# linum-uqam/ViT-OCM-WMSegmentation

Hardware: AMD Instinct MI355X
Metric: OCM tiles/s (224x224, ViT-S/16 attention-map inference) (higher is better)
Workload: dtype bf16x3

## Files before the change

vit-ocm-wmsegmentation_amd/csrc/engine.hip:

```cpp
#include <stdarg.h>
#include <stdio.h>
#include <string.h>

#include <atomic>
#include <mutex>
#include <string>
#include <vector>

#include "host_common.h"
#include "launch.h"
#include "dev_knobs.h"
#include "attn_plan.h"

static thread_local std::string g_err;

int ocm_fail(int code, const char *fmt, ...) {
    char buf[512];
    va_list ap;
    va_start(ap, fmt);
    vsnprintf(buf, sizeof buf, fmt, ap);
    va_end(ap);
    g_err = buf;
    return code;
}
// ... 330 lines not shown
    w.bytes = off;
    return w;
}

extern "C" size_t ocm_vit_workspace_bytes(const ocm_vit_t *h, int32_t batch, int32_t n_tokens) {
    if (!h || batch <= 0 || n_tokens <= 1) return 0;
    return carve(h, batch, n_tokens, nullptr).bytes;
}

static int check_ws(const ocm_vit *h, int batch, int n, void *ws, size_t ws_bytes) {
    if (!ws) return fail(OCM_ENOMEM, "workspace is null");
    if ((uintptr_t)ws & 255) return fail(OCM_EINVAL, "workspace must be 256-byte aligned");
    const size_t need = carve(h, batch, n, nullptr).bytes;
    if (ws_bytes < need) return fail(OCM_ENOMEM, "workspace too small: %zu < %zu bytes", ws_bytes, need);
    return OCM_OK;
}

static int run_attention(const ocm_vit *h, const Workspace &w, int batch, int n, bool attn_only, float *out_attn, float *out_qkv,
                         const int32_t *query_rows, int n_rows, float *out_rows, const char *qkv_w, const float *qkv_b,
                         const LnFold &ln, hipStream_t s) {
    const int H = h->H, np = ocm_n_pad_for(h->prec, n), pc = h->prec;
    const float scale = h->cfg.qk_scale;
    const bool want_v = !(attn_only && !out_qkv);
    if (!h->mfma_heads()) {
        float *qkv = out_qkv ? out_qkv : w.qkv32;
        { PROF(OCM_K_QKV, s); HIP_TRY(launch_qkv(pc, w.xn, qkv_w, qkv_b, nullptr, nullptr, nullptr, qkv, batch, n, np, H, h->hd, want_v, s, ln)); }
        { PROF(OCM_K_ATTN, s); HIP_TRY(launch_attention_generic(pc, qkv, attn_only ? nullptr : w.ctx, out_attn, query_rows, n_rows, out_rows, batch, n, H, h->hd, scale, s)); }
        return OCM_OK;
    }
    void *vt_dst = want_v ? w.vt : nullptr;
    { PROF(OCM_K_QKV, s); HIP_TRY(launch_qkv(pc, w.xn, qkv_w, qkv_b, w.q, w.k, vt_dst, out_qkv, batch, n, np, H, h->hd, want_v, s, ln)); }
    if (out_rows && !out_attn) { PROF(OCM_K_PROBS, s); HIP_TRY(launch_attention_rows(pc, w.q, w.k, query_rows, n_rows, out_rows, batch, n, np, H, scale, s, h->hd)); }
    if (attn_only && !out_attn) return OCM_OK;
    { PROF(OCM_K_ATTN, s); HIP_TRY(launch_attention(pc, w.q, w.k, w.vt, attn_only ? nullptr : w.ctx, out_attn ? w.lse : nullptr, batch, n, np, H, scale, s, h->hd, w.kpart, w.kpart_bytes)); }
    if (out_attn) {
        PROF(OCM_K_PROBS, s);
        HIP_TRY(launch_attention_probs(pc, w.q, w.k, w.lse, out_attn, batch, n, np, H, scale, s, h->hd, query_rows, n_rows, out_rows));
    }
    return OCM_OK;
}

static int run_block(const ocm_vit *h, int i, const Workspace &w, float *x, int batch, int n, bool attn_only,
                     float *out_attn, float *out_qkv, const int32_t *query_rows, int n_rows, float *out_rows,
                     hipStream_t s, bool xn_ready = false, const float *next_g = nullptr, const float *next_b = nullptr,
                     bool *xn_out = nullptr) {
    const BlockP &bp = h->blk[i];
    const int D = h->D, T = batch * n;
    const float eps = h->cfg.ln_eps;
    const int pc = h->prec, lnk = ln_kind_of_prec(pc);
    const long t128 = (long)((T + 127) / 128) * (D / 128);
    const int fuse_opt = h->opt[OCM_OPT_FUSE_LN];
    const bool fuse_ln = linear_resid_ln_supported(D) && fuse_opt != 1 && ((T >= 8192 && t128 < 512) || fuse_opt == 2);
    if (xn_out) *xn_out = false;
    if (!xn_ready) { PROF(OCM_K_LN, s); HIP_TRY(launch_layernorm(x, h->ptr<float>(bp.ln1_g), h->ptr<float>(bp.ln1_b), w.xn, lnk, T, D, eps, s)); }
    if (int rc = run_attention(h, w, batch, n, attn_only, out_attn, out_qkv, query_rows, n_rows, out_rows, h->ptr<char>(bp.qkv_w),
                               h->ptr<float>(bp.qkv_b), LnFold(), s))
        return rc;
    if (attn_only) return OCM_OK;
    if (fuse_ln) {
        PROF(OCM_K_PROJ, s);
        HIP_TRY(launch_linear_resid_ln(pc, w.ctx, h->ptr<char>(bp.proj_w), h->ptr<float>(bp.proj_b), x, x, h->ptr<float>(bp.ln2_g), h->ptr<float>(bp.ln2_b), w.xn, T, D, D, eps, s));
    } else {
        { PROF(OCM_K_PROJ, s); HIP_TRY(launch_linear(pc, w.ctx, h->ptr<char>(bp.proj_w), h->ptr<float>(bp.proj_b), x, x, T, D, D, OCM_EPI_BIAS_RESID_F32, s)); }
        { PROF(OCM_K_LN, s); HIP_TRY(launch_layernorm(x, h->ptr<float>(bp.ln2_g), h->ptr<float>(bp.ln2_b), w.xn, lnk, T, D, eps, s)); }
    }
    { PROF(OCM_K_FC1, s); HIP_TRY(launch_linear(pc, w.xn, h->ptr<char>(bp.fc1_w), h->ptr<float>(bp.fc1_b), nullptr, w.hid, T, h->M, D, OCM_EPI_BIAS_GELU_BF16, s)); }
    if (fuse_ln && next_g && next_b) {
        PROF(OCM_K_FC2, s);
        HIP_TRY(launch_linear_resid_ln(pc, w.hid, h->ptr<char>(bp.fc2_w), h->ptr<float>(bp.fc2_b), x, x, next_g, next_b, w.xn, T, D, h->M, eps, s));
        if (xn_out) *xn_out = true;
// ... 640 lines not shown
```

vit-ocm-wmsegmentation_amd/csrc/gemm_kernels.h:

```cpp
#pragma once
#include <type_traits>
#include "gemm_core.h"
#include "launch.h"
#include "gemm_plan.h"
#include "dev_knobs.h"

int ocm_wt_mask();

template <GemmTile T>
using CfgOf = GemmCfg<GEMM_TILES[T].bm, GEMM_TILES[T].bn, GEMM_TILES[T].waves_m, GEMM_TILES[T].waves_n, GEMM_TILES[T].mf16>;
typedef CfgOf<T128x128> Cfg128x128;
typedef CfgOf<T128x128q> Cfg128x128q;
typedef CfgOf<T128x128q16> Cfg128x128q16;
typedef CfgOf<T128x128m16> Cfg128x128m16;
typedef CfgOf<T160x128q16> Cfg160x128q16;
typedef CfgOf<T256x256m16> Cfg256x256m16;
typedef CfgOf<T64x128> Cfg64x128;
typedef CfgOf<T64x128w> Cfg64x128w;
typedef CfgOf<T64x64> Cfg64x64;
typedef CfgOf<T256x256> Cfg256x256;
typedef CfgOf<T256x128> Cfg256x128;
typedef CfgOf<T128x192> Cfg128x192;
typedef CfgOf<T128x96> Cfg128x96;

// ... 958 lines not shown
};

struct EpiPatch {
    static constexpr bool ROWTAB = false;
    const float *bias, *pos;
    float *x;
    int M, P, ntok, D;
    const float *mask, *mask_tok;
    StatsOut so;
    template <class Cfg>
    __device__ __forceinline__ void run(const float *C, int m0, int n0, const f32x2 *, const f32x2 *) const {
        constexpr int BM = Cfg::BM, BN = Cfg::BN, NT = Cfg::NT, CPR = BN / 4;
        if (so.stats) return run_stats<Cfg>(C, m0, n0);
#pragma unroll 4
        for (int q = threadIdx.x; q < BM * CPR; q += NT) {
            const int row = q / CPR, col = (q - row * CPR) * 4;
            const int m = m0 + row, n = n0 + col;
            if (m >= M || n >= D) continue;
            const int b = m / P, t = m - b * P;
            f32x4 v = *(const f32x4 *)(C + row * BN + col);
            if (mask) {
                const float w = mask[m], omw = 1.0f - w;
                const f32x4 tk = *(const f32x4 *)(mask_tok + n);
#pragma unroll
                for (int e = 0; e < 4; ++e) v[e] = v[e] * omw + tk[e] * w;
            }
            v += *(const f32x4 *)(pos + (int64_t)(1 + t) * D + n);
            *(f32x4 *)(x + ((int64_t)b * ntok + 1 + t) * D + n) = v;
        }
    }
    template <class Cfg>
    __device__ __forceinline__ void run_stats(const float *C, int m0, int n0) const {
        constexpr int BM = Cfg::BM, BN = Cfg::BN, NT = Cfg::NT, CPR = BN / 4;
        static_assert((BM * CPR) % NT == 0 && CPR <= 32 && (CPR & (CPR - 1)) == 0, "CPR lanes of one wave half own a row");
        const int sl = threadIdx.x & (CPR - 1), col = sl * 4, n = n0 + col;
        const bool nok = n < D;
        const int nc = min(n, D - 4);
#pragma unroll 1
        for (int row = threadIdx.x / CPR; row < BM; row += NT / CPR) {
            const int m = m0 + row;
            const bool ok = nok && m < M;
            const int mc = min(m, M - 1);
            const int b = mc / P, t = mc - b * P;
            f32x4 v = *(const f32x4 *)(C + row * BN + col);
            if (mask) {
                const float w = mask[mc], omw = 1.0f - w;
                const f32x4 tk = *(const f32x4 *)(mask_tok + nc);
#pragma unroll
                for (int e = 0; e < 4; ++e) v[e] = v[e] * omw + tk[e] * w;
            }
            v += *(const f32x4 *)(pos + (int64_t)(1 + t) * D + nc);
            const int64_t xrow = (int64_t)b * ntok + 1 + t;
            const float sh = so.tok_shift ? so.tok_shift[1 + t] : 0.f;
            float s1 = 0.f, s2 = 0.f;
            if (ok) {
                *(f32x4 *)(x + xrow * D + n) = v;
                if (so.shift && n0 == 0 && sl == 0) so.shift[xrow] = sh;
                v -= sh;
                bf16x4 hi, lo;
                split4(v, hi, lo);
                char *g = (char *)so.xs + xrow * D * 4 + sp_off(n);
                *(bf16x4 *)g = hi;
                *(bf16x4 *)(g + 64) = lo;
                s1 = (v[0] + v[1]) + (v[2] + v[3]);
                s2 = fmaf(v[0], v[0], fmaf(v[1], v[1], fmaf(v[2], v[2], v[3] * v[3])));
            }
#pragma unroll
            for (int o = CPR / 2; o > 0; o >>= 1) {
                s1 += __shfl_xor(s1, o, 64);
                s2 += __shfl_xor(s2, o, 64);
            }
            if (m < M && sl < BN / 64 && n0 + 64 * sl < D) {
                const f32x2 val = {sl ? 0.f : s1, sl ? 0.f : s2};
                *((f32x2 *)so.stats + xrow * (D >> 6) + (n0 >> 6) + sl) = val;
            }
        }
    }
};

template <class E>
hipError_t launch_patch_e(const PatchArgs &pa, const E *w, const float *bias, const float *pos, float *x, int dim,
                                 hipStream_t s, const StatsOut &so) {
    const int P = pa.hp * pa.wp, M = pa.batch * P, K = pa.chans * pa.p * pa.p;
    PatchLoader<E> al{pa.image, pa.sb, pa.sc, pa.sy, pa.origins, P, pa.wp, pa.p, pa.p * pa.p};
    EpiPatch epi{bias, pos, x, M, P, P + 1, dim, pa.mask, pa.mask_tok, so};
    if (K % Elem<E>::KROW) return hipErrorInvalidValue;
    const int ks = gemm_ct_steps<KsLinearReg>(K / Elem<E>::KROW);
    if constexpr (Elem<E>::MODE == 2)
        if (dim % 128 == 0 && M > 64 && M <= 1024) return launch_gemm<Cfg64x128w, E, false>(al, w, K, M, dim, K, epi, s, ks);
    if (dim % 128 == 0 && M > 64) return launch_gemm<Cfg64x128, E, false>(al, w, K, M, dim, K, epi, s, ks);
    return launch_gemm<Cfg64x64, E, false>(al, w, K, M, dim, K, epi, s, ks);
}
```

vit-ocm-wmsegmentation_amd/csrc/kernels_attn.hip:

```cpp
#include <stdlib.h>

#include "launch.h"

#define LOG2E 1.4426950408889634f
int ocm_wt_mask();
#include "dev_knobs.h"
#include "attn_plan.h"
#define OCM_VMCNT_ATTN(n) asm volatile("s_waitcnt vmcnt(%0)" ::"n"(n) : "memory")

#ifndef OCM_DEFER_MAX
#define OCM_DEFER_MAX 8.0f
#endif
__device__ __forceinline__ float defer_max_update(float &m, float cand) {
    if (__any(cand > m + OCM_DEFER_MAX)) {
        const float mn = fmaxf(m, cand);
        const float alpha = fast_exp2(m - mn);
        m = mn;
        return alpha;
    }
    return 1.0f;
}

template <bool WANT_O, int HD = 64>
__global__ __launch_bounds__(256, HD == 64 ? 3 : 2) void attn_fwd_kernel(const bf16 *__restrict__ Q, const bf16 *__restrict__ Kk,
// ... 531 lines not shown
#pragma unroll
            for (int c = 0; c < 4; ++c) {
                const f32x4 kf = *(const f32x4 *)(Kb + (int64_t)key * HD + 32 * hf + 16 * h + 4 * c);
#pragma unroll
                for (int e = 0; e < 4; ++e) S = mfma32f(qf[hf][c][e], kf[e], S);
            }
        if (kt * 32 + r < N) {
#pragma unroll
            for (int e = 0; e < 16; ++e) {
                const int qrow = q0 + acc_row32(e, h);
                if (qrow < N) out[(int64_t)qrow * N + kt * 32 + r] = fast_exp2(S[e] * scale2 - lr[e]);
            }
        }
    }
}

#ifdef OCM_GEMM_STAMPS
__device__ unsigned long long g_astamps[1024 * 8 * 16];
extern "C" int ocm_debug_stamps_attn(unsigned long long *host, int n) {
    return (int)hipMemcpyFromSymbol(host, HIP_SYMBOL(g_astamps), (size_t)n * 8);
}
#define ASTAMP(k)                                                                                                    \
    do {                                                                                                             \
        const unsigned wg_ = blockIdx.y * gridDim.x + blockIdx.x;                                                    \
        if ((threadIdx.x & 63) == 0 && wg_ < 1024 && (k) < 16)                                                       \
            g_astamps[(wg_ * 8 + (threadIdx.x >> 6 & 7)) * 16 + (k)] = __builtin_readcyclecounter();                 \
    } while (0)
#define ASTAMP_RT(k)                                                                                                 \
    do {                                                                                                             \
        const unsigned wg_ = blockIdx.y * gridDim.x + blockIdx.x;                                                    \
        if ((threadIdx.x & 63) == 0 && wg_ < 1024)                                                                   \
            g_astamps[(wg_ * 8 + (threadIdx.x >> 6 & 7)) * 16 + (k)] = wall_clock64();                               \
    } while (0)
#else
#define ASTAMP(k) ((void)0)
#define ASTAMP_RT(k) ((void)0)
#endif


template <int NQ>
__device__ __forceinline__ void x3_load_q(const char *qp, int h, bf16x8 (&qh)[NQ], bf16x8 (&ql)[NQ]) {
#pragma unroll
    for (int s = 0; s < NQ; ++s) {
        const char *p = qp + (s >> 1) * 128 + ((s & 1) * 16 + 8 * h) * 2;
        qh[s] = *(const bf16x8 *)p;
        ql[s] = *(const bf16x8 *)(p + 64);
    }
}

template <int HD, int NW, int KP, int VP>
__device__ __forceinline__ void x3_piece_offsets(int lane, int wave, int npad, int (&voffK)[KP], int (&voffV)[VP ? VP : 1]) {
    const int lrow = lane >> 3, slot = lane & 7;
#pragma unroll
    for (int j = 0; j < KP; ++j) {
        const int pc = j * NW + wave, rho = (pc & 3) * 8 + lrow;
        voffK[j] = rho * (HD * 4) + (pc >> 2) * 128 + ((slot ^ ((rho >> 1) & 7)) << 4);
    }
#pragma unroll
    for (int j = 0; j < VP; ++j) {
        const int rho = (j * NW + wave) * 8 + lrow;
        voffV[j] = rho * npad * 4 + ((slot ^ ((rho >> 1) & 7)) << 4);
    }
}
#if defined(__HIP_DEVICE_COMPILE__)
typedef __attribute__((address_space(3))) void *lds_ptr;
template <int HD>
__device__ __forceinline__ auto x3_tile_rsrc(const char *base, int npad) {
    return __builtin_amdgcn_make_buffer_rsrc((void *)base, 0, (unsigned)(npad * HD * 4), 0x00020000);
}
// ... 197 lines not shown
    }
    if (qrow < N) {
        if (lse2 && h == 0) lse2[(int64_t)bh * N + qrow] = m + __log2f(lt);
        if (WANT_O) {
            const float inv = 1.0f / lt;
            const int b = bh / H, head = bh - b * H;
            char *dst = ctx + ((int64_t)b * N + qrow) * (H * HD) * 4 + head * (HD * 4);
#pragma unroll
            for (int db = 0; db < ND; ++db)
#pragma unroll
                for (int g = 0; g < 4; ++g) {
                    f32x4 o;
#pragma unroll
                    for (int e = 0; e < 4; ++e) o[e] = O[db][4 * g + e] * inv;
                    bf16x4 oh, ol;
                    split4(o, oh, ol);
                    char *p = dst + db * 128 + (8 * g + 4 * h) * 2;
                    if (wt) {
                        const f32x2 dh = __builtin_bit_cast(f32x2, oh), dl = __builtin_bit_cast(f32x2, ol);
                        asm volatile("global_store_dwordx2 %0, %1, off sc1\n\ts_nop 1" ::"v"(p), "v"(dh) : "memory");
                        asm volatile("global_store_dwordx2 %0, %1, off sc1\n\ts_nop 1" ::"v"(p + 64), "v"(dl) : "memory");
                    } else {
                        *(bf16x4 *)p = oh;
                        *(bf16x4 *)(p + 64) = ol;
                    }
                }
        }
    }
    ASTAMP(15);
    ASTAMP_RT(13);
}


template <bool WANT_O>
__global__ __launch_bounds__(256, 3) void attn_fwd_x3_pp_kernel(const char *__restrict__ Q, const char *__restrict__ Kk,
                                                               const char *__restrict__ Vt, char *__restrict__ ctx,
                                                               float *__restrict__ lse2, int N, int npad, int H, float scale2) {
    constexpr int NW = 4, HD = 64, KB = HD * 128, KP = 8 / NW, VP = WANT_O ? 8 / NW : 0;
    __shared__ __attribute__((aligned(1024))) char smem[6 * KB];
    const int tid = threadIdx.x, lane = tid & 63;
    const int wave = __builtin_amdgcn_readfirstlane(tid >> 6);
    const int r = lane & 31, h = lane >> 5;
    int qblk, bh;
    xcd_remap2(qblk, bh);
    const int q0 = (qblk * NW + wave) * 32;
    const bool active = q0 < N;
    const char *Qb = Q + (int64_t)bh * npad * (HD * 4);
    const char *Kb = Kk + (int64_t)bh * npad * (HD * 4);
    const char *Vb = Vt + (int64_t)bh * HD * npad * 4;
    const int nt = (N + 31) >> 5;

    bf16x8 qh[4], ql[4];
    x3_load_q(Qb + (int64_t)min(q0 + r, N - 1) * (HD * 4), h, qh, ql);
    int voffK[KP], voffV[VP ? VP : 1];
    x3_piece_offsets<HD, NW, KP, VP>(lane, wave, npad, voffK, voffV);
#if defined(__HIP_DEVICE_COMPILE__)
    const auto rsK = x3_tile_rsrc<HD>(Kb, npad), rsV = x3_tile_rsrc<HD>(Vb, npad);
#define OCM_PP_DMA_K(t, slot)                                                                                        \
    do {                                                                                                             \
        _Pragma("unroll") for (int j = 0; j < KP; ++j)                                                               \
            __builtin_amdgcn_raw_ptr_buffer_load_lds(rsK, (lds_ptr)(smem + (slot) * KB + (j * NW + wave) * 1024), 16, \
                                                     voffK[j], (t) * (32 * HD * 4), 0, 0);                           \
    } while (0)
#define OCM_PP_DMA_V(t, slot)                                                                                              \
    do {                                                                                                                   \
        _Pragma("unroll") for (int j = 0; j < VP; ++j)                                                                     \
            __builtin_amdgcn_raw_ptr_buffer_load_lds(rsV, (lds_ptr)(smem + (3 + (slot)) * KB + (j * NW + wave) * 1024), 16, \
                                                     voffV[j], (t) * 128, 0, 0);                                           \
    } while (0)
#else
#define OCM_PP_DMA_K(t, slot) (void)0
#define OCM_PP_DMA_V(t, slot) (void)0
#endif
    OCM_PP_DMA_K(0, 0);
    if (nt > 1) OCM_PP_DMA_K(1, 1);
    if (WANT_O) OCM_PP_DMA_V(0, 0);
    if (nt > 2) OCM_PP_DMA_K(2, 2);
    if (WANT_O && nt > 1) OCM_PP_DMA_V(1, 1);
    __builtin_amdgcn_s_waitcnt(0x0F70);
    auto block_barrier = [&]() {
        __builtin_amdgcn_sched_barrier(0);
        asm volatile("s_waitcnt lgkmcnt(0)" ::: "memory");
        __builtin_amdgcn_s_barrier();
        asm volatile("" ::: "memory");
        __builtin_amdgcn_sched_barrier(0);
    };
    block_barrier();

    f32x16 O[2], S;
    bf16x8 ph[2], pl[2];
#pragma unroll
    for (int e = 0; e < 16; ++e) O[0][e] = O[1][e] = S[e] = 0.f;
#pragma unroll
    for (int s2 = 0; s2 < 2; ++s2)
#pragma unroll
        for (int e = 0; e < 8; ++e) ph[s2][e] = pl[s2][e] = (bf16)0.f;
    float m = -INFINITY, l = 0.f;
    const int pr = pi_row(r);
    const int first_pad = N - (nt - 1) * 32;

    auto qk = [&](int ks) {
        const char *Kt = smem + ks * KB;
#pragma unroll
        for (int e = 0; e < 16; ++e) S[e] = 0.f;
#pragma unroll
        for (int s = 0; s < 4; ++s) {
            const char *kp = Kt + (s >> 1) * 4096;
            const bf16x8 kh = *(const bf16x8 *)(kp + lds_off(pr, (s & 1) * 2 + h));
            const bf16x8 kl = *(const bf16x8 *)(kp + lds_off(pr, 4 + (s & 1) * 2 + h));
            S = mfma32x3(kh, kl, qh[s], ql[s], S);
        }
    };
    auto Mblk = [&](int vs, int ks, bool more) {
        if (WANT_O) {
            const char *Vtile = smem + (3 + vs) * KB;
#pragma unroll
            for (int s2 = 0; s2 < 2; ++s2)
#pragma unroll
                for (int db = 0; db < 2; ++db) {
                    const char *vp = Vtile + db * 32 * 128;
                    const bf16x8 vh = *(const bf16x8 *)(vp + lds_off(r, 2 * s2 + h));
                    const bf16x8 vl = *(const bf16x8 *)(vp + lds_off(r, 4 + 2 * s2 + h));
                    O[db] = mfma32x3(vh, vl, ph[s2], pl[s2], O[db]);
                }
        }
        if (more) qk(ks);
    };
    auto Vblk = [&](bool last_of_seq) {
        if (last_of_seq && first_pad < 32) x3_mask_pad_keys(S, first_pad, h);
        const float alpha = x3_softmax(S, scale2, m, l);
        if (WANT_O) {
            x3_rescale(O, alpha);
#pragma unroll
            for (int s2 = 0; s2 < 2; ++s2) x3_split_p(S, s2, ph[s2], pl[s2]);
        }
    };

    if (active) {
        qk(0);
        Vblk(nt == 1);
    }
    block_barrier();

    int s0 = 0, s1 = 1;
    for (int kt = 0; kt < nt; ++kt) {
        const int s2n = s1 == 2 ? 0 : s1 + 1;
        if (kt + 3 < nt) OCM_PP_DMA_K(kt + 3, s0);
        if (WANT_O && kt + 2 < nt) OCM_PP_DMA_V(kt + 2, s2n);
        const bool last = kt + 1 == nt;
        if (WANT_O && last && first_pad < 32) {
            x3_zero_pad_keys<HD, 64>(smem + (3 + s0) * KB, tid >> 2, tid & 3, first_pad);
            block_barrier();
        }
        if (active) {
            Mblk(s0, s1, !last);
            if (!last) Vblk(kt + 2 == nt);
        }
        if (kt + 3 < nt)
            OCM_VMCNT_ATTN(KP + VP);
        else if (WANT_O && kt + 2 < nt)
            OCM_VMCNT_ATTN(VP);
        else
            OCM_VMCNT_ATTN(0);
        block_barrier();
        s0 = s1;
        s1 = s2n;
    }
#undef OCM_PP_DMA_K
#undef OCM_PP_DMA_V

    if (!active) return;
    const float lt = l + __shfl_xor(l, 32, 64);
    const int qrow = q0 + r;
    if (lse2 && h == 0 && qrow < N) lse2[(int64_t)bh * N + qrow] = m + __log2f(lt);
    if (WANT_O) {
        const float inv = 1.0f / lt;
        const int b = bh / H, head = bh - b * H;
        char *dst = ctx + ((int64_t)b * N + min(qrow, N - 1)) * (H * HD) * 4 + head * (HD * 4);
#pragma unroll
        for (int db = 0; db < 2; ++db)
#pragma unroll
            for (int g = 0; g < 4; g += 2) {
                f32x4 oa, ob;
#pragma unroll
                for (int e = 0; e < 4; ++e) {
                    oa[e] = O[db][4 * g + e] * inv;
                    ob[e] = O[db][4 * g + 4 + e] * inv;
                }
                bf16x4 ah, al, bhh, bl;
                split4(oa, ah, al);
                split4(ob, bhh, bl);
                uint2 ahu = __builtin_bit_cast(uint2, ah), alu = __builtin_bit_cast(uint2, al);
                uint2 bhu = __builtin_bit_cast(uint2, bhh), blu = __builtin_bit_cast(uint2, bl);
                auto sw = [](unsigned &x, unsigned &y) {
                    const auto rr = __builtin_amdgcn_permlane32_swap(x, y, false, false);
                    x = rr[0];
                    y = rr[1];
                };
                sw(ahu.x, bhu.x);
                sw(ahu.y, bhu.y);
                sw(alu.x, blu.x);
                sw(alu.y, blu.y);
                if (qrow < N) {
                    char *p = dst + db * 128 + (8 * g + 8 * h) * 2;
                    *(uint4 *)p = make_uint4(ahu.x, ahu.y, bhu.x, bhu.y);
                    *(uint4 *)(p + 64) = make_uint4(alu.x, alu.y, blu.x, blu.y);
                }
            }
    }
}

template <bool WANT_O>
__global__ __launch_bounds__(256) void attn_fwd_x3_ws_kernel(const char *__restrict__ Q, const char *__restrict__ Kk,
                                                            const char *__restrict__ Vt, char *__restrict__ ctx,
                                                            float *__restrict__ lse2, int N, int npad, int H, float scale2) {
    constexpr int HD = 64, KB = HD * 128, SLOT = 2 * KB;
    extern __shared__ __attribute__((aligned(1024))) char smem[];
    const int tid = threadIdx.x, lane = tid & 63;
    const int wave = __builtin_amdgcn_readfirstlane(tid >> 6);
    const int r = lane & 31, h = lane >> 5;
    const int qt = blockIdx.x, bh = blockIdx.y;
    const int q0 = qt * 32;
    const char *Qb = Q + (int64_t)bh * npad * (HD * 4);
    const char *Kb = Kk + (int64_t)bh * npad * (HD * 4);
    const char *Vb = Vt + (int64_t)bh * HD * npad * 4;
    const int nt = (N + 31) >> 5;
    char *mine = smem + wave * 2 * SLOT;

    bf16x8 qh[4], ql[4];
    x3_load_q(Qb + (int64_t)min(q0 + r, N - 1) * (HD * 4), h, qh, ql);
    int voffK[8], voffV[WANT_O ? 8 : 1];
    x3_piece_offsets<HD, 1, 8, WANT_O ? 8 : 0>(lane, 0, npad, voffK, voffV);
#if defined(__HIP_DEVICE_COMPILE__)
    const auto rsK = x3_tile_rsrc<HD>(Kb, npad), rsV = x3_tile_rsrc<HD>(Vb, npad);
#define OCM_WS_DMA(t, sl)                                                                                              \
    do {                                                                                                               \
        char *st_ = mine + (sl) * SLOT;                                                                                \
        _Pragma("unroll") for (int pc = 0; pc < 8; ++pc)                                                               \
            __builtin_amdgcn_raw_ptr_buffer_load_lds(rsK, (lds_ptr)(st_ + pc * 1024), 16, voffK[pc], (t) * (32 * HD * 4), 0, 0); \
        if (WANT_O) {                                                                                                  \
            _Pragma("unroll") for (int pc = 0; pc < 8; ++pc)                                                           \
                __builtin_amdgcn_raw_ptr_buffer_load_lds(rsV, (lds_ptr)(st_ + KB + pc * 1024), 16, voffV[pc], (t) * 128, 0, 0); \
// ... 194 lines not shown
#pragma unroll
    for (int e = 0; e < 16; ++e) lr[e] = lse2[(int64_t)bh * N + min(q0 + acc_row32(e, h), N - 1)];
    float *out = attn + (int64_t)bh * N * N;
    const int nkt = (N + 31) >> 5, per = (nkt + (int)gridDim.z - 1) / (int)gridDim.z;
    const int kt0 = (int)blockIdx.z * per, ktiles = min(nkt, kt0 + per);
    if (kt0 >= ktiles) return;
    bf16x8 kh[NQ], kl[NQ], nh[NQ], nl[NQ];
    loadrow(Kb, min(kt0 * 32 + r, N - 1), kh, kl);
    for (int kt = kt0; kt < ktiles; ++kt) {
        if (kt + 1 < ktiles) loadrow(Kb, min((kt + 1) * 32 + r, N - 1), nh, nl);
        f32x16 S;
#pragma unroll
        for (int e = 0; e < 16; ++e) S[e] = 0.f;
#pragma unroll
        for (int s = 0; s < NQ; ++s) S = mfma32x3(qh[s], ql[s], kh[s], kl[s], S);
        const int key = kt * 32 + r;
        if (key < N) {
#pragma unroll
            for (int e = 0; e < 16; ++e) {
                const int qrow = q0 + acc_row32(e, h);
                if (qrow < N) out[(int64_t)qrow * N + key] = fast_exp2(S[e] * scale2 - lr[e]);
            }
        }
#pragma unroll
        for (int s = 0; s < NQ; ++s) {
            kh[s] = nh[s];
            kl[s] = nl[s];
        }
    }
}

constexpr int PROBS_FOLD_ROWS = 8;

__global__ __launch_bounds__(256) void attn_probs_x3_span_kernel(const char *__restrict__ Q, const char *__restrict__ Kk,
                                                                 const float *__restrict__ lse2, float *__restrict__ attn,
                                                                 int N, int npad, float scale2,
                                                                 const int32_t *__restrict__ query_rows, int n_rows,
                                                                 float *__restrict__ rows) {
    constexpr int HD = 64, NQ = HD / 16, ROWB = HD * 4, PITCH = ROWB + 16, REGION = 32 * PITCH, TILEB = 32 * ROWB;
    __shared__ __attribute__((aligned(16))) char smem[4 * REGION];
    const int tid = threadIdx.x, lane = tid & 63, wave = tid >> 6;
    const int r = lane & 31, h = lane >> 5;
    int qblk, bh;
    xcd_remap2(qblk, bh);
    const int q0 = qblk * 32, nq = min(32, N - q0);
    const int nkt = (N + 31) >> 5;
    const char *Qb = Q + ((int64_t)bh * npad + q0) * ROWB;
    const char *Kb = Kk + (int64_t)bh * npad * ROWB;
    f32x4 qraw[2], kraw[2][8];
#pragma unroll
    for (int i = 0; i < 2; ++i) qraw[i] = *(const f32x4 *)(Qb + (i * 256 + tid) * 16);
#pragma unroll
    for (int t = 0; t < 2; ++t)
        if (wave + 4 * t < nkt) {
#pragma unroll
            for (int i = 0; i < 8; ++i) kraw[t][i] = *(const f32x4 *)(Kb + (int64_t)(wave + 4 * t) * TILEB + (i * 64 + lane) * 16);
        }
    float lr[16];
#pragma unroll
    for (int e = 0; e < 16; ++e) lr[e] = lse2[(int64_t)bh * N + min(q0 + acc_row32(e, h), N - 1)];
    auto stage = [&](char *region, int piece, const f32x4 &v) {
        *(f32x4 *)(region + (piece >> 4) * PITCH + (piece & 15) * 16) = v;
    };
    auto fragments = [&](const char *region, bf16x8(&hi)[NQ], bf16x8(&lo)[NQ]) {
        const char *rp = region + r * PITCH;
#pragma unroll
        for (int s = 0; s < NQ; ++s) {
            const char *p = rp + (s >> 1) * 128 + ((s & 1) * 16 + 8 * h) * 2;
            hi[s] = *(const bf16x8 *)p;
            lo[s] = *(const bf16x8 *)(p + 64);
        }
    };
    bf16x8 qh[NQ], ql[NQ];
#pragma unroll
    for (int i = 0; i < 2; ++i) stage(smem, i * 256 + tid, qraw[i]);
    lds_barrier();
    fragments(smem, qh, ql);
    lds_barrier();
    char *mine = smem + wave * REGION;
    float pr[2][16];
#pragma unroll
    for (int t = 0; t < 2; ++t) {
        const bool have = wave + 4 * t < nkt;
        if (have) {
#pragma unroll
            for (int i = 0; i < 8; ++i) stage(mine, i * 64 + lane, kraw[t][i]);
        }
        lds_barrier();
        if (have) {
            bf16x8 kh[NQ], kl[NQ];
            fragments(mine, kh, kl);
            f32x16 S;
#pragma unroll
            for (int e = 0; e < 16; ++e) S[e] = 0.f;
#pragma unroll
            for (int s = 0; s < NQ; ++s) S = mfma32x3(qh[s], ql[s], kh[s], kl[s], S);
#pragma unroll
            for (int e = 0; e < 16; ++e) pr[t][e] = fast_exp2(S[e] * scale2 - lr[e]);
        }
        lds_barrier();
    }
    float *span = attn + ((int64_t)bh * N + q0) * N;
    const int shift = (int)(((uintptr_t)span >> 2) & 3);
    float *img = (float *)smem + shift;
#pragma unroll
    for (int t = 0; t < 2; ++t) {
        const int key = (wave + 4 * t) * 32 + r;
        if (key < N) {
#pragma unroll
            for (int e = 0; e < 16; ++e) {
                const int row = acc_row32(e, h);
                if (row < nq) img[row * N + key] = pr[t][e];
            }
        }
    }
    lds_barrier();
    const int len = nq * N;
    const int lead = min((4 - shift) & 3, len), nvec = (len - lead) >> 2, tail = lead + 4 * nvec;
    if (tid < lead) span[tid] = img[tid];
    for (int i = tid; i < nvec; i += 256) *(f32x4 *)(span + lead + 4 * i) = *(const f32x4 *)(img + lead + 4 * i);
    if (tid < len - tail) span[tail + tid] = img[tail + tid];
    if (rows) {
        for (int i = 0; i < n_rows; ++i) {
            const int query = query_rows ? query_rows[i] : 0;
            if (query < q0 || query >= q0 + nq) continue;
            float *dst = rows + ((int64_t)bh * n_rows + i) * (N - 1);
            const float *src = img + (query - q0) * N + 1;
            for (int j = tid; j < N - 1; j += 256) dst[j] = src[j];
        }
    }
}


__device__ __forceinline__ void store_ctx1(int prec, char *rowp, int col, float v) {
    if (prec == 0) {
        *(bf16 *)(rowp + col * 2) = (bf16)v;
    } else if (prec == 1) {
        *(float *)(rowp + col * 4) = v;
    } else {
        bf16 hi, lo;
        split1(v, hi, lo);
        *(bf16 *)(rowp + sp_off(col)) = hi;
        *(bf16 *)(rowp + sp_off(col) + 64) = lo;
    }
}

__global__ __launch_bounds__(256) void attn_generic_kernel(const float *__restrict__ qkv, char *__restrict__ ctx,
                                                           float *__restrict__ attn, const int32_t *__restrict__ query_rows,
                                                           int n_rows, float *__restrict__ rows, int B, int H, int N,
// ... 143 lines not shown
                kern<<<grid, block, 0, s>>>(Q, K, V, (char *)ctx, lse2, n_tokens, n_pad, heads, scale2, 0, nullptr);
            } else {
                auto kern = ctx ? attn_fwd_x3_dma_kernel<true, 8, 2> : attn_fwd_x3_dma_kernel<false, 8, 2>;
                kern<<<grid, block, 0, s>>>(Q, K, V, (char *)ctx, lse2, n_tokens, n_pad, heads, scale2, (ocm_wt_mask() >> 4) & 1,
                                            nullptr);
            }
            break;
        case ATTN_X3_DMA_KSPLIT: {
            auto kern = ctx ? attn_fwd_x3_dma_kernel<true, 8, 2, 64, 3, true> : attn_fwd_x3_dma_kernel<false, 8, 2, 64, 3, true>;
            kern<<<grid, block, 0, s>>>(Q, K, V, (char *)ctx, lse2, n_tokens, n_pad, heads, scale2, 0, ksplit_ws);
            if (hipError_t e = hipGetLastError(); e != hipSuccess) return e;
            const int64_t rows = (int64_t)batch * heads * n_tokens;
            attn_merge_x3_kernel<64><<<dim3((unsigned)((rows + 15) / 16)), dim3(256), 0, s>>>(
                ksplit_ws, p.kslices, (char *)ctx, lse2, batch * heads, n_tokens, heads);
            break;
        }
    }
    return hipGetLastError();
}

template <int HD>
static hipError_t launch_probs_hd(int prec, const void *q, const void *k, const float *lse2, float *attn, int n_tokens, int n_pad,
                                  float scale2, dim3 grid, dim3 gridz, hipStream_t s) {
    const dim3 block(256);
    if (prec == 2)
        attn_probs_x3_kernel<HD><<<gridz, block, 0, s>>>((const char *)q, (const char *)k, lse2, attn, n_tokens, n_pad, scale2);
    else if (prec)
        attn_probs_f32_kernel<HD><<<grid, block, 0, s>>>((const float *)q, (const float *)k, lse2, attn, n_tokens, n_pad, scale2);
    else
        attn_probs_kernel<HD><<<grid, block, 0, s>>>((const bf16 *)q, (const bf16 *)k, lse2, attn, n_tokens, n_pad, scale2);
    return hipGetLastError();
}

hipError_t launch_attention_probs(int prec, const void *q, const void *k, const float *lse2, float *attn, int batch,
                                  int n_tokens, int n_pad, int heads, float scale, hipStream_t s, int head_dim,
                                  const int32_t *query_rows, int n_rows, float *rows) {
    if (head_dim != 64 && head_dim != 128) return hipErrorInvalidValue;
    const int qtiles = (n_tokens + 31) / 32;
    const dim3 grid((qtiles + 3) / 4, batch * heads);
    const int wgs = (int)(grid.x * grid.y), ktiles = qtiles;
    int nz = wgs >= 256 ? 1 : min(ktiles, min(16, (512 + wgs - 1) / wgs));
    if (OCM_KNOB(2) > 0) nz = min(ktiles, OCM_KNOB(2));
    const dim3 gridz(grid.x, grid.y, nz);
    if (n_rows <= 0) rows = nullptr;
    bool folded = false;
    hipError_t e;
    if (prec == 2 && head_dim == 64 && n_tokens <= 255 && n_pad % 32 == 0 && n_pad >= n_tokens) {
        folded = rows && n_rows <= PROBS_FOLD_ROWS;
        attn_probs_x3_span_kernel<<<dim3(qtiles, batch * heads), dim3(256), 0, s>>>(
            (const char *)q, (const char *)k, lse2, attn, n_tokens, n_pad, scale * LOG2E, query_rows, n_rows, folded ? rows : nullptr);
        e = hipGetLastError();
    } else if (head_dim == 128) {
        e = launch_probs_hd<128>(prec, q, k, lse2, attn, n_tokens, n_pad, scale * LOG2E, grid, gridz, s);
    } else {
        e = launch_probs_hd<64>(prec, q, k, lse2, attn, n_tokens, n_pad, scale * LOG2E, grid, gridz, s);
    }
    if (e != hipSuccess || !rows || folded) return e;
    return launch_rows_from_probs(attn, query_rows, n_rows, rows, batch, n_tokens, heads, s);
}

__device__ __forceinline__ void load8(const bf16 *rowp, int c, float (&o)[8]) {
    const bf16x8 t = *(const bf16x8 *)(rowp + c * 8);
#pragma unroll
    for (int e = 0; e < 8; ++e) o[e] = (float)t[e];
}
__device__ __forceinline__ void load8(const float *rowp, int c, float (&o)[8]) {
    const f32x4 a = *(const f32x4 *)(rowp + c * 8), b = *(const f32x4 *)(rowp + c * 8 + 4);
#pragma unroll
    for (int e = 0; e < 4; ++e) {
        o[e] = a[e];
        o[4 + e] = b[e];
    }
}
__device__ __forceinline__ void load8(const sp32 *rowp, int c, float (&o)[8]) {
    const char *p = (const char *)rowp + sp_off(c * 8);
    const bf16x8 hi = *(const bf16x8 *)p, lo = *(const bf16x8 *)(p + 64);
#pragma unroll
    for (int e = 0; e < 8; ++e) o[e] = (float)hi[e] + (float)lo[e];
}

template <class E, int HD>
__global__ __launch_bounds__(64) void attn_rows_kernel(const E *__restrict__ Q, const E *__restrict__ Kk,
                                                       const int32_t *__restrict__ query_rows, int n_rows,
// ... 117 lines not shown
```

vit-ocm-wmsegmentation_amd/csrc/launch.h:

```cpp
#pragma once
#include <atomic>
#include "common.h"
#include "gemm_plan.h"

typedef std::atomic<unsigned long long> OptinMask;
static inline hipError_t lds_optin(const void *kern, int bytes, OptinMask &done) {
    int dev = 0;
    if (hipError_t e = hipGetDevice(&dev); e != hipSuccess) return e;
    const unsigned long long bit = 1ull << (dev & 63);
    if (done.load(std::memory_order_acquire) & bit) return hipSuccess;
    const hipError_t e = hipFuncSetAttribute(kern, hipFuncAttributeMaxDynamicSharedMemorySize, bytes);
    if (e == hipSuccess) done.fetch_or(bit, std::memory_order_release);
    return e;
}

hipError_t launch_layernorm(const float *x, const float *gamma, const float *beta, void *y, int out_kind,
                            int64_t rows, int dim, float eps, hipStream_t s);
static inline int ln_kind_of_prec(int prec) { return prec == 0 ? 1 : prec == 1 ? 0 : 2; }
hipError_t launch_cast_bf16(const float *src, bf16 *dst, size_t count, hipStream_t s);
hipError_t launch_cast_split(const float *src, void *dst, size_t count, hipStream_t s);
hipError_t launch_merge_split(const void *src, float *dst, size_t count, hipStream_t s);
hipError_t launch_fold_split(const float *src, void *dst, int D, int C, int pp, hipStream_t s);
hipError_t launch_fold_cast_bf16(const float *src, bf16 *dst, int D, int C, int pp, hipStream_t s);
hipError_t launch_fold_f32(const float *src, float *dst, int D, int C, int pp, hipStream_t s);
// ... 22 lines not shown
                                 int n_tokens, int dim, hipStream_t s, float *shift = nullptr, float *tok_shift = nullptr,
                                 const float *pe_bias = nullptr);
hipError_t launch_fold_ln(const float *W, const float *gamma, const float *beta, const float *bias, void *Wf, float *cvec,
                          float *dvec, int N, int K, hipStream_t s);

hipError_t launch_linear(int prec, const void *a, const void *w, const float *bias, const float *resid, void *out, int M,
                         int N, int K, int epilogue, hipStream_t s, const LnFold &ln = LnFold(),
                         const StatsOut &so = StatsOut());
bool linear_resid_ln_supported(int D);
hipError_t launch_linear_resid_ln(int prec, const void *a, const void *w, const float *bias, const float *resid, float *x,
                                  const float *gamma, const float *beta, void *xn, int M, int D, int K, float eps,
                                  hipStream_t s);
hipError_t launch_qkv(int prec, const void *a, const void *w, const float *bias, void *q, void *k, void *vt,
                      float *qkv_f32, int batch, int n_tokens, int n_pad, int heads, int head_dim, bool want_v,
                      hipStream_t s, const LnFold &ln = LnFold());
hipError_t launch_attention_generic(int prec, const float *qkv, void *ctx, float *attn, const int32_t *query_rows,
                                    int n_rows, float *rows, int batch, int n_tokens, int heads, int head_dim, float scale,
                                    hipStream_t s);
struct PatchArgs {
    const float *image;
    int64_t sb, sc, sy;
    const int32_t *origins;
    int batch, hp, wp, p, chans;
    const float *mask = nullptr;
    const float *mask_tok = nullptr;
};
hipError_t launch_patch_embed(int prec, const PatchArgs &pa, const void *w, const float *bias, const float *pos,
                              float *x, int dim, hipStream_t s, const StatsOut &so = StatsOut());

hipError_t launch_attention(int prec, const void *q, const void *k, const void *vt, void *ctx, float *lse2, int batch,
                            int n_tokens, int n_pad, int heads, float scale, hipStream_t s, int head_dim = 64,
                            float *ksplit_ws = nullptr, size_t ksplit_bytes = 0);
size_t attention_ksplit_bytes(int prec, int batch, int n_tokens, int heads, int head_dim);
hipError_t launch_attention_probs(int prec, const void *q, const void *k, const float *lse2, float *attn, int batch,
                                  int n_tokens, int n_pad, int heads, float scale, hipStream_t s, int head_dim = 64,
                                  const int32_t *query_rows = nullptr, int n_rows = 0, float *rows = nullptr);
hipError_t launch_rows_from_probs(const float *attn, const int32_t *query_rows, int n_rows, float *rows, int batch,
                                  int n_tokens, int heads, hipStream_t s);
hipError_t launch_attention_rows(int prec, const void *q, const void *k, const int32_t *query_rows, int n_rows,
                                 float *rows, int batch, int n_tokens, int n_pad, int heads, float scale, hipStream_t s,
                                 int head_dim = 64);
hipError_t launch_attention_map(const float *attn, float *maps, int b, int heads, int n_tokens, int query, int hf,
                                int wf, int p, hipStream_t s);

hipError_t launch_tile_postprocess(const float *rows, float *maps, int tiles, int heads, int n_rows, int pixels,
                                   hipStream_t s);
hipError_t launch_bilinear_up(const float *src, float *dst, int tiles, int h, int w, int scale, hipStream_t s);
hipError_t launch_nearest_up(const float *src, float *dst, int tiles, int h, int w, int rep, hipStream_t s);
hipError_t launch_stitch(const float *crops, float *out, const double *ramp, int n, int window, int stride,
                         hipStream_t s);
hipError_t launch_normalize_u8(const float *img, size_t count, float *part, uint8_t *out,
                               unsigned long long *hist256, hipStream_t s);
hipError_t launch_threshold_u8(const uint8_t *img, uint8_t *mask, size_t count, int thresh, hipStream_t s);
hipError_t launch_tokens_to_fmap(const float *y, float *out, int batch, int n_tokens, int dim, hipStream_t s);
hipError_t launch_pixel_shuffle(const float *lin, float *out, int batch, int hp, int wp, int c_out, int sh, hipStream_t s);
hipError_t launch_head_mean(const float *rows, float *maps, int tiles, int heads, int n_rows, int pixels, hipStream_t s);
hipError_t launch_image_to_gray_u8(const float *img, int64_t stride_c, int chans, size_t count, uint8_t *out,
                                   unsigned long long *hist256, hipStream_t s);
hipError_t launch_blend_u8(const uint8_t *img, const uint8_t *att, size_t count, double alpha, double one_minus_alpha,
                           uint8_t *out, unsigned long long *hist256, hipStream_t s);

hipError_t launch_stitch_image_u8(const float *image, int64_t sc, int64_t sy, int chans, int H, int W, uint8_t *out,
                                  const double *ramp, int n, int window, int stride, unsigned long long *hist256,
                                  hipStream_t s);
hipError_t launch_weighted_u8(const float *heat, const uint8_t *img, size_t count, float *part, uint8_t *result,
                              uint8_t *att_u8, unsigned long long *hist_res, unsigned long long *hist_att, hipStream_t s);
// ... 38 lines not shown
```

vit-ocm-wmsegmentation_amd/csrc/common.h:

```cpp
#pragma once
#include <hip/hip_runtime.h>
#include <stddef.h>
#include <stdint.h>

typedef __bf16 bf16;
typedef __bf16 bf16x2 __attribute__((ext_vector_type(2)));
typedef __bf16 bf16x4 __attribute__((ext_vector_type(4)));
typedef __bf16 bf16x8 __attribute__((ext_vector_type(8)));
typedef float f32x2 __attribute__((ext_vector_type(2)));
typedef float f32x4 __attribute__((ext_vector_type(4)));
typedef float f32x16 __attribute__((ext_vector_type(16)));

#define OCM_WAVE 64
#define OCM_HEAD_DIM 64

__device__ __forceinline__ int acc_row32(int reg, int h) { return (reg & 3) + 8 * (reg >> 2) + 4 * h; }

__device__ __forceinline__ int lds_off(int row, int chunk) {
    return row * 128 + ((chunk ^ ((row >> 1) & 7)) << 4);
}

__device__ __forceinline__ void lds_barrier() {
    __builtin_amdgcn_fence(__ATOMIC_RELEASE, "workgroup", "local");
    __builtin_amdgcn_s_barrier();
// ... 72 lines not shown
#if defined(__HIP_DEVICE_COMPILE__)
    typedef short s16x4 __attribute__((ext_vector_type(4)));
    typedef __attribute__((address_space(3))) s16x4 *lds_s16x4;
    const s16x4 a = __builtin_amdgcn_ds_read_tr16_b64_v4i16((lds_s16x4)p);
    const s16x4 b = __builtin_amdgcn_ds_read_tr16_b64_v4i16((lds_s16x4)(p + 4 * 64));
    typedef short s16x8 __attribute__((ext_vector_type(8)));
    const s16x8 v = {a[0], a[1], a[2], a[3], b[0], b[1], b[2], b[3]};
    return __builtin_bit_cast(bf16x8, v);
#else
    return bf16x8{};
#endif
}

template <int ACCL>
__device__ __forceinline__ int acc_rpos(int e, int lane) {
    return ACCL ? 16 * (e >> 3) + 4 * ((lane >> 4) & 3) + (e & 3) : acc_row32(e, lane >> 5);
}
template <int ACCL>
__device__ __forceinline__ int acc_cpos(int e, int lane) {
    return ACCL ? 16 * ((e >> 2) & 1) + (lane & 15) : (lane & 31);
}

__device__ __forceinline__ int xcd_remap(int bid, int nwg) {
    const int q = nwg >> 3, r = nwg & 7, x = bid & 7;
    return (x < r ? x * (q + 1) : r * (q + 1) + (x - r) * q) + (bid >> 3);
}

__device__ __forceinline__ void xcd_remap2(int &bx, int &by) {
    const int id = xcd_remap(blockIdx.y * gridDim.x + blockIdx.x, gridDim.x * gridDim.y);
    by = id / (int)gridDim.x;
    bx = id - by * (int)gridDim.x;
}

__device__ __forceinline__ float fast_exp2(float x) { return __builtin_amdgcn_exp2f(x); }

__device__ __forceinline__ int key_of_reg(int reg, int h) {
    return (reg & 3) + 4 * ((reg >> 2) & 1) + 8 * h + 16 * (reg >> 3);
}
__device__ __forceinline__ int pi_row(int r) {
    return (r & ~12) | ((r & 4) << 1) | ((r & 8) >> 1);
}

__device__ __forceinline__ float erf_as(float x) {
    const float ax = fabsf(x);
    const float t = __builtin_amdgcn_rcpf(fmaf(0.3275911f, ax, 1.0f));
    float p = fmaf(1.061405429f, t, -1.453152027f);
    p = fmaf(p, t, 1.421413741f);
    p = fmaf(p, t, -0.284496736f);
    p = fmaf(p, t, 0.254829592f);
    const float e = __builtin_amdgcn_exp2f(-1.4426950408889634f * ax * ax);
    const float r = fmaf(-p * t, e, 1.0f);
    return copysignf(r, x);
}
__device__ __forceinline__ f32x2 gelu_erf2(f32x2 x) {
    const f32x2 ax = {fabsf(x[0]), fabsf(x[1])};
    const f32x2 den = ax * 0.2316418882f + 1.0f;
    const f32x2 t = {__builtin_amdgcn_rcpf(den[0]), __builtin_amdgcn_rcpf(den[1])};
    f32x2 p = t * 0.5307027145f + (-0.7265760135f);
    p = p * t + 0.7107068705f;
    p = p * t + (-0.142248368f);
    p = p * t + 0.127414796f;
    p = p * t;
    const f32x2 u = x * 0.8493218003f;
    const f32x2 nu2 = -(u * u);
    const f32x2 e = {__builtin_amdgcn_exp2f(nu2[0]), __builtin_amdgcn_exp2f(nu2[1])};
    const f32x2 g = ax * p * e;
// ... 6 lines not shown
```

Measured before the change: 29520.

## Compute softmax stats inside probs kernel and add wide patch-embed tile

The bf16x3 attention-probs kernel can now compute each row's max and sum itself in LDS and normalise there, instead of reading a log-sum-exp written by the flash-attention kernel. In attention-only mode this lets the full attention pass be skipped entirely, and otherwise the LSE write is dropped. Separately, patch embedding for dim 384 with large M gets a 64x384 tile with its own k-step table, and the stats epilogue is split into 128-column segments to support it. The in-kernel softmax adds per-row reductions and register use, and only handles up to 256 tokens.

```diff
diff --git a/vit-ocm-wmsegmentation_amd/csrc/engine.hip b/vit-ocm-wmsegmentation_amd/csrc/engine.hip
--- a/vit-ocm-wmsegmentation_amd/csrc/engine.hip
+++ b/vit-ocm-wmsegmentation_amd/csrc/engine.hip
@@ -386,10 +386,12 @@
     { PROF(OCM_K_QKV, s); HIP_TRY(launch_qkv(pc, w.xn, qkv_w, qkv_b, w.q, w.k, vt_dst, out_qkv, batch, n, np, H, h->hd, want_v, s, ln)); }
     if (out_rows && !out_attn) { PROF(OCM_K_PROBS, s); HIP_TRY(launch_attention_rows(pc, w.q, w.k, query_rows, n_rows, out_rows, batch, n, np, H, scale, s, h->hd)); }
     if (attn_only && !out_attn) return OCM_OK;
-    { PROF(OCM_K_ATTN, s); HIP_TRY(launch_attention(pc, w.q, w.k, w.vt, attn_only ? nullptr : w.ctx, out_attn ? w.lse : nullptr, batch, n, np, H, scale, s, h->hd, w.kpart, w.kpart_bytes)); }
+    const bool own_stats = out_attn && attention_probs_own_stats(pc, h->hd, n, np);
+    float *lse = out_attn && !own_stats ? w.lse : nullptr;
+    if (!(attn_only && own_stats)) { PROF(OCM_K_ATTN, s); HIP_TRY(launch_attention(pc, w.q, w.k, w.vt, attn_only ? nullptr : w.ctx, lse, batch, n, np, H, scale, s, h->hd, w.kpart, w.kpart_bytes)); }
     if (out_attn) {
         PROF(OCM_K_PROBS, s);
-        HIP_TRY(launch_attention_probs(pc, w.q, w.k, w.lse, out_attn, batch, n, np, H, scale, s, h->hd, query_rows, n_rows, out_rows));
+        HIP_TRY(launch_attention_probs(pc, w.q, w.k, lse, out_attn, batch, n, np, H, scale, s, h->hd, query_rows, n_rows, out_rows));
     }
     return OCM_OK;
 }
diff --git a/vit-ocm-wmsegmentation_amd/csrc/gemm_kernels.h b/vit-ocm-wmsegmentation_amd/csrc/gemm_kernels.h
--- a/vit-ocm-wmsegmentation_amd/csrc/gemm_kernels.h
+++ b/vit-ocm-wmsegmentation_amd/csrc/gemm_kernels.h
@@ -1014,6 +1014,17 @@
     template <class Cfg>
     __device__ __forceinline__ void run_stats(const float *C, int m0, int n0) const {
         constexpr int BM = Cfg::BM, BN = Cfg::BN, NT = Cfg::NT, CPR = BN / 4;
+        if constexpr (CPR > 32) {
+            static_assert(BN % 128 == 0, "segments of 128 columns");
+#pragma unroll 1
+            for (int seg = 0; seg < BN / 128; ++seg) run_stats_seg<BM, BN, 128, NT>(C + seg * 128, m0, n0 + seg * 128);
+        } else {
+            run_stats_seg<BM, BN, BN, NT>(C, m0, n0);
+        }
+    }
+    template <int BM, int LDC, int SN, int NT>
+    __device__ __forceinline__ void run_stats_seg(const float *C, int m0, int n0) const {
+        constexpr int BN = SN, CPR = BN / 4;
         static_assert((BM * CPR) % NT == 0 && CPR <= 32 && (CPR & (CPR - 1)) == 0, "CPR lanes of one wave half own a row");
         const int sl = threadIdx.x & (CPR - 1), col = sl * 4, n = n0 + col;
         const bool nok = n < D;
@@ -1024,7 +1035,7 @@
             const bool ok = nok && m < M;
             const int mc = min(m, M - 1);
             const int b = mc / P, t = mc - b * P;
-            f32x4 v = *(const f32x4 *)(C + row * BN + col);
+            f32x4 v = *(const f32x4 *)(C + row * LDC + col);
             if (mask) {
                 const float w = mask[mc], omw = 1.0f - w;
                 const f32x4 tk = *(const f32x4 *)(mask_tok + nc);
@@ -1060,6 +1071,10 @@
     }
 };
 
+struct KsPatchRows {
+    static constexpr int n = 2, v[n] = {6, 24};
+};
+
 template <class E>
 hipError_t launch_patch_e(const PatchArgs &pa, const E *w, const float *bias, const float *pos, float *x, int dim,
                                  hipStream_t s, const StatsOut &so) {
@@ -1068,8 +1083,11 @@
     EpiPatch epi{bias, pos, x, M, P, P + 1, dim, pa.mask, pa.mask_tok, so};
     if (K % Elem<E>::KROW) return hipErrorInvalidValue;
     const int ks = gemm_ct_steps<KsLinearReg>(K / Elem<E>::KROW);
-    if constexpr (Elem<E>::MODE == 2)
+    if constexpr (Elem<E>::MODE == 2) {
         if (dim % 128 == 0 && M > 64 && M <= 1024) return launch_gemm<Cfg64x128w, E, false>(al, w, K, M, dim, K, epi, s, ks);
+        if (dim == 384 && M > 127 * 64)
+            return launch_gemm<CfgOf<T64x384w>, E, false, KsPatchRows>(al, w, K, M, dim, K, epi, s, gemm_ct_steps<KsPatchRows>(K / Elem<E>::KROW));
+    }
     if (dim % 128 == 0 && M > 64) return launch_gemm<Cfg64x128, E, false>(al, w, K, M, dim, K, epi, s, ks);
     return launch_gemm<Cfg64x64, E, false>(al, w, K, M, dim, K, epi, s, ks);
 }
diff --git a/vit-ocm-wmsegmentation_amd/csrc/kernels_attn.hip b/vit-ocm-wmsegmentation_amd/csrc/kernels_attn.hip
--- a/vit-ocm-wmsegmentation_amd/csrc/kernels_attn.hip
+++ b/vit-ocm-wmsegmentation_amd/csrc/kernels_attn.hip
@@ -1289,6 +1289,7 @@
 
 constexpr int PROBS_FOLD_ROWS = 8;
 
+template <bool OWN_STATS>
 __global__ __launch_bounds__(256) void attn_probs_x3_span_kernel(const char *__restrict__ Q, const char *__restrict__ Kk,
                                                                  const float *__restrict__ lse2, float *__restrict__ attn,
                                                                  int N, int npad, float scale2,
@@ -1314,8 +1315,10 @@
             for (int i = 0; i < 8; ++i) kraw[t][i] = *(const f32x4 *)(Kb + (int64_t)(wave + 4 * t) * TILEB + (i * 64 + lane) * 16);
         }
     float lr[16];
-#pragma unroll
-    for (int e = 0; e < 16; ++e) lr[e] = lse2[(int64_t)bh * N + min(q0 + acc_row32(e, h), N - 1)];
+    if constexpr (!OWN_STATS) {
+#pragma unroll
+        for (int e = 0; e < 16; ++e) lr[e] = lse2[(int64_t)bh * N + min(q0 + acc_row32(e, h), N - 1)];
+    }
     auto stage = [&](char *region, int piece, const f32x4 &v) {
         *(f32x4 *)(region + (piece >> 4) * PITCH + (piece & 15) * 16) = v;
     };
@@ -1353,7 +1356,12 @@
 #pragma unroll
             for (int s = 0; s < NQ; ++s) S = mfma32x3(qh[s], ql[s], kh[s], kl[s], S);
 #pragma unroll
-            for (int e = 0; e < 16; ++e) pr[t][e] = fast_exp2(S[e] * scale2 - lr[e]);
+            for (int e = 0; e < 16; ++e) {
+                if constexpr (OWN_STATS)
+                    pr[t][e] = S[e] * scale2;
+                else
+                    pr[t][e] = fast_exp2(S[e] * scale2 - lr[e]);
+            }
         }
         lds_barrier();
     }
@@ -1372,6 +1380,37 @@
         }
     }
     lds_barrier();
+    if constexpr (OWN_STATS) {
+        const int row = (tid >> 5) + 8 * ((tid >> 3) & 3), j = tid & 7;
+        if (row < nq) {
+            float *rp = img + row * N;
+            float v[32];
+            float m = -INFINITY;
+#pragma unroll
+            for (int i = 0; i < 32; ++i) {
+                const int c = j + 8 * i;
+                v[i] = c < N ? rp[c] : -INFINITY;
+                m = fmaxf(m, v[i]);
+            }
+#pragma unroll
+            for (int o = 1; o < 8; o <<= 1) m = fmaxf(m, __shfl_xor(m, o, 64));
+            float l = 0.f;
+#pragma unroll
+            for (int i = 0; i < 32; ++i) {
+                v[i] = fast_exp2(v[i] - m);
+                l += v[i];
+            }
+#pragma unroll
+            for (int o = 1; o < 8; o <<= 1) l += __shfl_xor(l, o, 64);
+            const float inv = 1.0f / l;
+#pragma unroll
+            for (int i = 0; i < 32; ++i) {
+                const int c = j + 8 * i;
+                if (c < N) rp[c] = v[i] * inv;
+            }
+        }
+        lds_barrier();
+    }
     const int len = nq * N;
     const int lead = min((4 - shift) & 3, len), nvec = (len - lead) >> 2, tail = lead + 4 * nvec;
     if (tid < lead) span[tid] = img[tid];
@@ -1581,6 +1620,10 @@
     return hipGetLastError();
 }
 
+bool attention_probs_own_stats(int prec, int head_dim, int n_tokens, int n_pad) {
+    return prec == 2 && head_dim == 64 && n_tokens <= 255 && n_pad % 32 == 0 && n_pad >= n_tokens;
+}
+
 hipError_t launch_attention_probs(int prec, const void *q, const void *k, const float *lse2, float *attn, int batch,
                                   int n_tokens, int n_pad, int heads, float scale, hipStream_t s, int head_dim,
                                   const int32_t *query_rows, int n_rows, float *rows) {
@@ -1594,10 +1637,12 @@
     if (n_rows <= 0) rows = nullptr;
     bool folded = false;
     hipError_t e;
+    if (!lse2 && !attention_probs_own_stats(prec, head_dim, n_tokens, n_pad)) return hipErrorInvalidValue;
     if (prec == 2 && head_dim == 64 && n_tokens <= 255 && n_pad % 32 == 0 && n_pad >= n_tokens) {
         folded = rows && n_rows <= PROBS_FOLD_ROWS;
-        attn_probs_x3_span_kernel<<<dim3(qtiles, batch * heads), dim3(256), 0, s>>>(
-            (const char *)q, (const char *)k, lse2, attn, n_tokens, n_pad, scale * LOG2E, query_rows, n_rows, folded ? rows : nullptr);
+        auto kern = lse2 ? attn_probs_x3_span_kernel<false> : attn_probs_x3_span_kernel<true>;
+        kern<<<dim3(qtiles, batch * heads), dim3(256), 0, s>>>((const char *)q, (const char *)k, lse2, attn, n_tokens, n_pad,
+                                                               scale * LOG2E, query_rows, n_rows, folded ? rows : nullptr);
         e = hipGetLastError();
     } else if (head_dim == 128) {
         e = launch_probs_hd<128>(prec, q, k, lse2, attn, n_tokens, n_pad, scale * LOG2E, grid, gridz, s);
diff --git a/vit-ocm-wmsegmentation_amd/csrc/launch.h b/vit-ocm-wmsegmentation_amd/csrc/launch.h
--- a/vit-ocm-wmsegmentation_amd/csrc/launch.h
+++ b/vit-ocm-wmsegmentation_amd/csrc/launch.h
@@ -78,6 +78,7 @@
                             int n_tokens, int n_pad, int heads, float scale, hipStream_t s, int head_dim = 64,
                             float *ksplit_ws = nullptr, size_t ksplit_bytes = 0);
 size_t attention_ksplit_bytes(int prec, int batch, int n_tokens, int heads, int head_dim);
+bool attention_probs_own_stats(int prec, int head_dim, int n_tokens, int n_pad);
 hipError_t launch_attention_probs(int prec, const void *q, const void *k, const float *lse2, float *attn, int batch,
                                   int n_tokens, int n_pad, int heads, float scale, hipStream_t s, int head_dim = 64,
                                   const int32_t *query_rows = nullptr, int n_rows = 0, float *rows = nullptr);
```

Result: no change. 29520 (-0.0%).

## Overlap attention prologue loads with first tile and rotate block placement

Applied to the files above, without the earlier changes.

The prologue of the pipelined x3 attention kernel now waits only for the first K/V tiles to arrive before the first barrier, not for all prefetches, so tile 0 compute overlaps the remaining loads. Out-of-range tile prefetches are clamped rather than skipped, which keeps the vmcnt counts fixed. Block-to-tile mapping is also rotated per head (OCM_PP_ROT) so concurrently running blocks on an XCD touch different query blocks. Timestamp instrumentation is added but compiled out by default. The clamped loads may issue redundant DMA for short sequences.

```diff
diff --git a/vit-ocm-wmsegmentation_amd/csrc/common.h b/vit-ocm-wmsegmentation_amd/csrc/common.h
--- a/vit-ocm-wmsegmentation_amd/csrc/common.h
+++ b/vit-ocm-wmsegmentation_amd/csrc/common.h
@@ -128,6 +128,12 @@
     bx = id - by * (int)gridDim.x;
 }
 
+__device__ __forceinline__ void xcd_remap2_rot(int &bx, int &by, int period) {
+    xcd_remap2(bx, by);
+    const int gx = (int)gridDim.x;
+    bx = (bx + by * gx / period) % gx;
+}
+
 __device__ __forceinline__ float fast_exp2(float x) { return __builtin_amdgcn_exp2f(x); }
 
 __device__ __forceinline__ int key_of_reg(int reg, int h) {
diff --git a/vit-ocm-wmsegmentation_amd/csrc/kernels_attn.hip b/vit-ocm-wmsegmentation_amd/csrc/kernels_attn.hip
--- a/vit-ocm-wmsegmentation_amd/csrc/kernels_attn.hip
+++ b/vit-ocm-wmsegmentation_amd/csrc/kernels_attn.hip
@@ -587,9 +587,24 @@
         if ((threadIdx.x & 63) == 0 && wg_ < 1024)                                                                   \
             g_astamps[(wg_ * 8 + (threadIdx.x >> 6 & 7)) * 16 + (k)] = wall_clock64();                               \
     } while (0)
+__device__ unsigned g_astamp_place[1024 * 4];
+extern "C" int ocm_debug_stamps_attn_place(unsigned *host, int n) {
+    return (int)hipMemcpyFromSymbol(host, HIP_SYMBOL(g_astamp_place), (size_t)n * 4);
+}
+#define ASTAMP_PLACE(lx, ly)                                                                                         \
+    do {                                                                                                             \
+        const unsigned wg_ = blockIdx.y * gridDim.x + blockIdx.x;                                                    \
+        if (threadIdx.x == 0 && wg_ < 1024) {                                                                        \
+            g_astamp_place[wg_ * 4 + 0] = __builtin_amdgcn_s_getreg(20 | (31 << 11));                                \
+            g_astamp_place[wg_ * 4 + 1] = __builtin_amdgcn_s_getreg(4 | (31 << 11));                                 \
+            g_astamp_place[wg_ * 4 + 2] = (unsigned)(lx);                                                            \
+            g_astamp_place[wg_ * 4 + 3] = (unsigned)(ly);                                                            \
+        }                                                                                                            \
+    } while (0)
 #else
 #define ASTAMP(k) ((void)0)
 #define ASTAMP_RT(k) ((void)0)
+#define ASTAMP_PLACE(lx, ly) ((void)0)
 #endif
 
 
@@ -853,6 +868,9 @@
 }
 
 
+#ifndef OCM_PP_ROT
+#define OCM_PP_ROT 32
+#endif
 template <bool WANT_O>
 __global__ __launch_bounds__(256, 3) void attn_fwd_x3_pp_kernel(const char *__restrict__ Q, const char *__restrict__ Kk,
                                                                const char *__restrict__ Vt, char *__restrict__ ctx,
@@ -862,8 +880,15 @@
     const int tid = threadIdx.x, lane = tid & 63;
     const int wave = __builtin_amdgcn_readfirstlane(tid >> 6);
     const int r = lane & 31, h = lane >> 5;
+    ASTAMP(0);
+    ASTAMP_RT(12);
     int qblk, bh;
+#if OCM_PP_ROT
+    xcd_remap2_rot(qblk, bh, OCM_PP_ROT);
+#else
     xcd_remap2(qblk, bh);
+#endif
+    ASTAMP_PLACE(qblk, bh);
     const int q0 = (qblk * NW + wave) * 32;
     const bool active = q0 < N;
     const char *Qb = Q + (int64_t)bh * npad * (HD * 4);
@@ -893,12 +918,6 @@
 #define OCM_PP_DMA_K(t, slot) (void)0
 #define OCM_PP_DMA_V(t, slot) (void)0
 #endif
-    OCM_PP_DMA_K(0, 0);
-    if (nt > 1) OCM_PP_DMA_K(1, 1);
-    if (WANT_O) OCM_PP_DMA_V(0, 0);
-    if (nt > 2) OCM_PP_DMA_K(2, 2);
-    if (WANT_O && nt > 1) OCM_PP_DMA_V(1, 1);
-    __builtin_amdgcn_s_waitcnt(0x0F70);
     auto block_barrier = [&]() {
         __builtin_amdgcn_sched_barrier(0);
         asm volatile("s_waitcnt lgkmcnt(0)" ::: "memory");
@@ -906,7 +925,32 @@
         asm volatile("" ::: "memory");
         __builtin_amdgcn_sched_barrier(0);
     };
+#define OCM_PP_VMCNT_Q(n) __builtin_amdgcn_s_waitcnt(0x0F70 | (n))
+#if defined(OCM_ABL) && OCM_ABL == 16
+    OCM_PP_DMA_K(0, 0);
+    if (nt > 1) OCM_PP_DMA_K(1, 1);
+    if (WANT_O) OCM_PP_DMA_V(0, 0);
+    if (nt > 2) OCM_PP_DMA_K(2, 2);
+    if (WANT_O && nt > 1) OCM_PP_DMA_V(1, 1);
+    OCM_PP_VMCNT_Q(0);
+    ASTAMP(1);
     block_barrier();
+    ASTAMP(2);
+#else
+    const int t1 = min(1, nt - 1), t2 = min(2, nt - 1);
+    OCM_PP_DMA_K(0, 0);
+    OCM_PP_DMA_K(t1, 1);
+    if (WANT_O) OCM_PP_DMA_V(0, 0);
+    OCM_PP_DMA_K(t2, 2);
+    if (WANT_O) OCM_PP_DMA_V(t1, 1);
+#ifdef OCM_GEMM_STAMPS
+    OCM_PP_VMCNT_Q(3 * KP + 2 * VP);
+    ASTAMP(1);
+#endif
+    OCM_PP_VMCNT_Q(2 * KP + 2 * VP);
+    block_barrier();
+    ASTAMP(2);
+#endif
 
     f32x16 O[2], S;
     bf16x8 ph[2], pl[2];
@@ -961,6 +1005,10 @@
         qk(0);
         Vblk(nt == 1);
     }
+    ASTAMP(3);
+#if !defined(OCM_ABL) || OCM_ABL != 16
+    OCM_VMCNT_ATTN(KP + VP);
+#endif
     block_barrier();
 
     int s0 = 0, s1 = 1;
@@ -984,13 +1032,19 @@
         else
             OCM_VMCNT_ATTN(0);
         block_barrier();
+        if (kt < 8) ASTAMP(4 + kt);
         s0 = s1;
         s1 = s2n;
     }
 #undef OCM_PP_DMA_K
 #undef OCM_PP_DMA_V
-
-    if (!active) return;
+#undef OCM_PP_VMCNT_Q
+    ASTAMP(14);
+
+    if (!active) {
+        ASTAMP_RT(13);
+        return;
+    }
     const float lt = l + __shfl_xor(l, 32, 64);
     const int qrow = q0 + r;
     if (lse2 && h == 0 && qrow < N) lse2[(int64_t)bh * N + qrow] = m + __log2f(lt);
@@ -1029,6 +1083,8 @@
                 }
             }
     }
+    ASTAMP(15);
+    ASTAMP_RT(13);
 }
 
 template <bool WANT_O>
```

Result: no change. 27780 before, 27930 after (median of 6 runs) (+0.6%).
